# Multi-resolution-diffusion-recommender/SDRM

Hardware: AMD Instinct MI355X
Metric: denoising-steps/sec (train+sample) on ML-1M latents (higher is better)
Workload: dtype f32; 1 GPU; ML-1M/MLP shaped synthetic latents (C3/C4); latent=340, width=340, hidden_layers=1, global_batch=8192, n_sample=5429, step_mix=15 train : 78 sample per job cycle, rng=philox4x32-10 on device, sampler_row_chains=2, parallelism=user-sharded dp1, collectives=none

## Files before the change

### include/sdrm_hip_debug.h

```cpp
#ifndef SDRM_HIP_DEBUG_H
#define SDRM_HIP_DEBUG_H

#include "sdrm_hip.h"

#ifdef __cplusplus
extern "C" {
#endif

int sdrm_debug_device_check(const char* gcn_arch, int compute_units);

enum { SDRM_TILE_AUTO = -1, SDRM_TILE_COUNT = 5 };

int sdrm_debug_set_tile(sdrm_engine* e, int cfg);
int sdrm_debug_set_nt32_rows(sdrm_engine* e, int max_rows, int max_rows_train);
int sdrm_debug_set_skinny(sdrm_engine* e, int on);
int sdrm_debug_set_rowchain(sdrm_engine* e, int mode);
int sdrm_debug_set_rows48(sdrm_engine* e, int mode);
int sdrm_debug_set_rows48_split(sdrm_engine* e, int mode);
int sdrm_debug_rows48_split_available(const sdrm_engine* e);
int sdrm_debug_set_rows48_share(sdrm_engine* e, int on);
int sdrm_debug_set_sample_persist(sdrm_engine* e, int mode);
int sdrm_debug_split_skew(sdrm_engine* e, unsigned skew);
int sdrm_debug_set_wgrad_strips(sdrm_engine* e, int on);
int sdrm_debug_set_dgrad_rows(sdrm_engine* e, int mode);
int sdrm_debug_rowchain_available(const sdrm_engine* e);
int sdrm_debug_set_fused_reverse(sdrm_engine* e, int mode);
int sdrm_debug_set_chains(sdrm_engine* e, int chains);
int sdrm_debug_chains(const sdrm_engine* e);

int sdrm_debug_set_gradient_buckets(sdrm_engine* e, int buckets);

int sdrm_debug_philox_draws(sdrm_engine* e, uint64_t seed, uint32_t purpose, uint32_t step, int64_t row0, int rows, int quads,
                            float* normals, uint8_t* lowbits, void* stream);

void* sdrm_debug_comm_handle(const sdrm_engine* e);

int sdrm_debug_plan_wgrad(int rows, int n_out, int k_in, int* slices, int* rows_per_slice);

int sdrm_debug_gemm(int variant, int cfg, const float* A, const float* B, float* C, int M, int N, int K, void* stream);
int sdrm_debug_gemm_time(int variant, int cfg, int M, int N, int K, int reps, float* us_out, void* stream);

#ifdef __cplusplus
}
#endif
#endif
```

### sdrm_amd/_lib.py

```python
from __future__ import annotations

import ctypes as C
import os

from . import _build

_LIB = None

c_void_p, c_int, c_int64, c_uint64, c_float = C.c_void_p, C.c_int, C.c_int64, C.c_uint64, C.c_float


class TrainRandoms(C.Structure):
    _fields_ = [("noise", c_void_p), ("t", c_void_p), ("keep", c_void_p)]


class VaeDecoder(C.Structure):
    _fields_ = [("w1", c_void_p), ("b1", c_void_p), ("w2", c_void_p), ("b2", c_void_p), ("latent", c_int), ("hidden", c_int),
                ("n_items", c_int)]


class VaeEncoder(C.Structure):
    _fields_ = [("w1", c_void_p), ("b1", c_void_p), ("w2", c_void_p), ("b2", c_void_p), ("n_items", c_int), ("hidden", c_int),
                ("latent", c_int)]

# ... 74 lines not shown
    "sdrm_debug_set_skinny": (c_int, [c_void_p, c_int]),
    "sdrm_debug_set_rowchain": (c_int, [c_void_p, c_int]),
    "sdrm_debug_set_rows48": (c_int, [c_void_p, c_int]),
    "sdrm_debug_set_rows48_split": (c_int, [c_void_p, c_int]),
    "sdrm_debug_rows48_split_available": (c_int, [c_void_p]),
    "sdrm_debug_split_skew": (c_int, [c_void_p, C.c_uint32]),
    "sdrm_debug_set_sample_persist": (c_int, [c_void_p, c_int]),
    "sdrm_debug_set_rows48_share": (c_int, [c_void_p, c_int]),
    "sdrm_debug_rowchain_available": (c_int, [c_void_p]),
    "sdrm_debug_set_wgrad_strips": (c_int, [c_void_p, c_int]),
    "sdrm_debug_set_dgrad_rows": (c_int, [c_void_p, c_int]),
    "sdrm_debug_comm_handle": (c_void_p, [c_void_p]),
    "sdrm_debug_plan_wgrad": (c_int, [c_int, c_int, c_int, C.POINTER(c_int), C.POINTER(c_int)]),
    "sdrm_debug_gemm_time": (c_int, [c_int, c_int, c_int, c_int, c_int, c_int, C.POINTER(c_float), c_void_p]),
    "sdrm_debug_gemm": (c_int, [c_int, c_int, c_void_p, c_void_p, c_void_p, c_int, c_int, c_int, c_void_p]),
}

RNG_EXPLICIT, RNG_PHILOX = 0, 1
STATUS = {0: "SDRM_OK", -1: "SDRM_ERR_ARG", -2: "SDRM_ERR_SHAPE", -3: "SDRM_ERR_HIP", -4: "SDRM_ERR_STATE",
          -5: "SDRM_ERR_NOMEM", -6: "SDRM_ERR_RCCL", -7: "SDRM_ERR_DEVICE"}


def lib_path() -> str:
    return _build.LIB_PATH


def load(build_if_missing: bool = True):
    global _LIB
    if _LIB is not None:
        return _LIB
# ... 37 lines not shown
```

### sdrm_amd/csrc/gemm.h

```cpp
#pragma once
#include <hip/hip_runtime.h>
#include <stdint.h>

#include "bufres.h"

#include <type_traits>

#include "philox.h"
#include "select.h"

namespace sdrm {

typedef float f32x16 __attribute__((ext_vector_type(16)));

enum : int { LD_KCONTIG = 0, LD_MCONTIG = 1 };
enum : int { XF_NONE = 0, XF_PRELU = 1 };
enum : int {
  EPI_BIAS = 0,
  EPI_BIAS_TANH = 1,
  EPI_BIAS_TANH_G = 2,
  EPI_DPRELU = 3,
  EPI_SLAB = 4,
  EPI_PLAIN = 5,
  EPI_TANH_REV = 6,
// ... 23 lines not shown
  static constexpr int STAGE = STAGE_KMAJOR > STAGE_KMINOR ? STAGE_KMAJOR : STAGE_KMINOR;
  static_assert(WM_ * WN_ == 4, "4 waves per work-group");
  static_assert(MF_ == 32 || MF_ == 16, "MFMA tile edge");
  static_assert(TM >= 1 && TN >= 1, "wave tile must hold at least one MFMA tile");
};

template <int MF> struct AccT;
template <> struct AccT<32> { typedef float type __attribute__((ext_vector_type(16))); };
template <> struct AccT<16> { typedef float type __attribute__((ext_vector_type(4))); };

struct GemmArgs {
  const float* A; int lda; int limA;
  const float* B; int ldb; int limB;
  float* C; int ldc;
  int K;
  int kchunk;
  int tiles_n;
  int nblocks;
  int nsplits;
  uint32_t magic_tiles_n, magic_nblocks;
  const float* bias;
  const float* slopeA;
  const float* slopeB;
  const float* aux; int ldaux; const float* slopeE; float* slope_partial;
  size_t slab_stride; float* dbias; int dbias_stride;
  unsigned long long* stamps;
  int rows_valid, cols_valid;
  float* revX; float* revU; int rev_ldx, rev_s0, rev_n, rev_L, rev_step;
  float rev_c1, rev_sqrt_alpha, rev_sqrt_beta, rev_nd;
  uint32_t rev_seed_lo, rev_seed_hi, rev_call_id; int64_t rev_row0;
// ... 260 lines not shown
    if constexpr (PF_STATE) {
      const int rows_left = min(max(p.rev_n - p.rev_s0 - m0, 0), BM);
      const brsrc resX = make_brsrc(p.revX + (size_t)(p.rev_s0 + m0) * p.rev_ldx, (uint32_t)rows_left * (uint32_t)p.rev_ldx * 4u);
#pragma unroll
      for (int a = 0; a < TM; ++a)
#pragma unroll
        for (int b = 0; b < TN; ++b) {
          const int col = n0 + wn * (BN / Cfg::WN) + b * MF + l31;
          const int r0 = wm * (BM / Cfg::WM) + a * MF + 4 * lhi;
#pragma unroll
          for (int r = 0; r < NR; ++r)
            pf_x[a][b][r] = bload1a<COHA>(resX, (uint32_t)((r0 + ((MF == 32) ? (r & 3) + 8 * (r >> 2) : r)) * p.rev_ldx + col) * 4u, 0u);
        }
    }
  };
  const int aoffk = (wm * (BM / Cfg::WM) + l31) * LDK + ((MF == 32) ? (BK / 2) : 4) * lhi;
  const int boffk = (wn * (BN / Cfg::WN) + l31) * LDK + ((MF == 32) ? (BK / 2) : 4) * lhi;

  if constexpr (KM) {
    constexpr int NS = 4 * NQ;
    static_assert(NS >= 2 * NQ + 4, "not enough MFMA shadows for the pipeline pieces");
    float4 fa0[TM][NQ], fb0[TN][NQ], fa1[TM][NQ], fb1[TN][NQ];
    auto rd_all = [&](float4 (&fa)[TM][NQ], float4 (&fb)[TN][NQ], int stage) {
      const float* As = smem + stage * Cfg::STAGE;
      const float* Bs = As + BOFF;
#pragma unroll
      for (int q = 0; q < NQ; ++q) {
#pragma unroll
        for (int a = 0; a < TM; ++a) fa[a][q] = *reinterpret_cast<const float4*>(As + aoffk + MF * a * LDK + QSTEP * q);
#pragma unroll
        for (int b = 0; b < TN; ++b) fb[b][q] = *reinterpret_cast<const float4*>(Bs + boffk + MF * b * LDK + QSTEP * q);
      }
    };
    auto kstep = [&](auto active_tag, const float4 (&ca)[TM][NQ], const float4 (&cb)[TN][NQ], float4 (&na)[TM][NQ],
                     float4 (&nb)[TN][NQ], int rs, float4 (&xa)[NVA], float4 (&xb)[NVB], int ss, int li) {
      constexpr bool ACTIVE = decltype(active_tag)::value;
      const float* Ar = smem + rs * Cfg::STAGE;
      const float* Br = Ar + BOFF;
      float* Aw = smem + ss * Cfg::STAGE;
      const int k0 = kb + min(li, nt - 1) * BK;
#pragma unroll
      for (int sl = 0; sl < NS; ++sl) {
        const int q = sl >> 2, j = sl & 3;
        if constexpr (ACTIVE) {
#pragma unroll
          for (int a = 0; a < TM; ++a)
#pragma unroll
            for (int b = 0; b < TN; ++b) {
              const float av = j == 0 ? ca[a][q].x : j == 1 ? ca[a][q].y : j == 2 ? ca[a][q].z : ca[a][q].w;
              const float bv = j == 0 ? cb[b][q].x : j == 1 ? cb[b][q].y : j == 2 ? cb[b][q].z : cb[b][q].w;
              if constexpr (MF == 32) acc[a][b] = __builtin_amdgcn_mfma_f32_32x32x2f32(av, bv, acc[a][b], 0, 0, 0);
              else acc[a][b] = __builtin_amdgcn_mfma_f32_16x16x4f32(av, bv, acc[a][b], 0, 0, 0);
            }
        }
        if (sl < 2 * NQ) {
          if constexpr (ACTIVE) {
            const int rq = sl >> 1;
            if ((sl & 1) == 0) {
#pragma unroll
              for (int a = 0; a < TM; ++a) na[a][rq] = *reinterpret_cast<const float4*>(Ar + aoffk + MF * a * LDK + QSTEP * rq);
            } else {
#pragma unroll
              for (int b = 0; b < TN; ++b) nb[b][rq] = *reinterpret_cast<const float4*>(Br + boffk + MF * b * LDK + QSTEP * rq);
            }
          }
        } else if (sl == 2 * NQ) {
          if constexpr (XFA == XF_PRELU) prelu_regs<NVA>(xa, slopeA);
          else DIAG_ST((store_tile_km<XF_NONE, BM, LDK, BK>(Aw, xa, 0.f, tid)));
        } else if (sl == 2 * NQ + 1) {
          if constexpr (XFA == XF_PRELU) DIAG_ST((store_tile_km<XF_NONE, BM, LDK, BK>(Aw, xa, 0.f, tid)));
          DIAG_ST((store_tile_km<XFB, BN, LDK, BK>(Aw + BOFF, xb, slopeB, tid)));
        } else if (sl == 2 * NQ + 2) {
          DIAG_LD((load_tile<LOADA, BM, BK, COHA>(resA, voA, p.lda, k0 - kb, xa)));
        } else if (sl == 2 * NQ + 3) {
          DIAG_LD((load_tile<LOADB, BN, BK>(resB, voB, p.ldb, k0 - kb, xb)));
        }
        __builtin_amdgcn_sched_barrier(0);
      }
      DIAG_BAR();
    };
    if (nt > 0) {
      if constexpr (Cfg::PF == 2) {
        ld(ra0, rb0, 0);
        ld(ra1, rb1, 1);
#if defined(SDRM_STAMPS) && SDRM_STAMPS == 2
        t_ld = __builtin_amdgcn_s_memtime();
        __builtin_amdgcn_sched_barrier(0);
#endif
        epi_prefetch();
        if constexpr (EPI == EPI_TANH_REV) rev_draw();
        st(ra0, rb0, 0);
#if defined(SDRM_STAMPS) && SDRM_STAMPS == 2
        __builtin_amdgcn_sched_barrier(0);
        t_land = __builtin_amdgcn_s_memtime();
#endif
        ld(ra0, rb0, 2);
        st(ra1, rb1, 1);
        ld(ra1, rb1, 3);
      } else {
        ld(ra0, rb0, 0);
        epi_prefetch();
        if constexpr (EPI == EPI_TANH_REV) rev_draw();
        st(ra0, rb0, 0);
        ld(ra0, rb0, 1);
        st(ra0, rb0, 1);
        ld(ra0, rb0, 2);
      }
      __syncthreads();
#ifdef SDRM_STAMPS
      if (true) t_pro = __builtin_amdgcn_s_memtime();
#endif
      if (wave_active) rd_all(fa0, fb0, 0);
      __syncthreads();
      auto run = [&](auto tag) {
        int i = 0;
        for (; i + 1 < nt; i += 2) {
          if constexpr (Cfg::PF == 2) {
            kstep(tag, fa0, fb0, fa1, fb1, 1, ra0, rb0, 0, i + 4);
            kstep(tag, fa1, fb1, fa0, fb0, 0, ra1, rb1, 1, i + 5);
          } else {
            kstep(tag, fa0, fb0, fa1, fb1, 1, ra0, rb0, 0, i + 3);
            kstep(tag, fa1, fb1, fa0, fb0, 0, ra0, rb0, 1, i + 4);
          }
        }
        if (i < nt) kstep(tag, fa0, fb0, fa1, fb1, 1, ra0, rb0, 0, i + 4);
      };
      if (wave_active) run(std::true_type{});
      else run(std::false_type{});
    }
  } else {
    constexpr int G = BK / KG;
    static_assert(G >= 8, "pipeline pieces need 8 MFMA shadows");
    float ka0[TM][G], kb0[TN][G], ka1[TM][G], kb1[TN][G];
    auto col_sum = [&](int stage) {
      const float* As = smem + stage * Cfg::STAGE;
#pragma unroll
      for (int k = 0; k < BK; ++k) dbsum += As[k * LDA + tid];
    };
    auto kstep = [&](auto active_tag, const float (&ca)[TM][G], const float (&cb)[TN][G], float (&na)[TM][G],
                     float (&nb)[TN][G], int rs, float4 (&xa)[NVA], float4 (&xb)[NVB], int ss, int li, bool next_valid) {
// ... 224 lines not shown
```

### sdrm_amd/csrc/sdrm_hip.hip

```cpp
#include <hip/hip_runtime.h>

#include <algorithm>
#include <cmath>
#include <cstdio>
#include <cstdlib>
#include <cstring>
#include <mutex>
#include <set>
#include <string>
#include <type_traits>
#include <utility>
#include <vector>

#include "../../include/sdrm_hip.h"
#include "../../include/sdrm_hip_debug.h"
#include "compact.h"
#include "decode.h"
#include "elementwise.h"
#include "encode.h"
#include "exchange.h"
#include "feed.h"
#include "gemm.h"
#include "rank.h"
#include "rowchain.h"
// ... 332 lines not shown
    default: return launch_gemm_cfg<Cfg0, LA, LB, XA, XB, EPI>(a, M, N, splits, st, pr);
  }
}

template <int XA, int EPI>
hipError_t gemm_forward(GemmArgs a, const float* A, int lda, const float* Wc, int ldw, int M, int N, int K,
                        hipStream_t st, Prof pr, int cfg) {
  a.A = A; a.lda = lda; a.limA = M;
  a.B = Wc; a.ldb = ldw; a.limB = N;
  a.K = K; a.kchunk = K;
  return launch_gemm<LD_KCONTIG, LD_KCONTIG, XA, XF_NONE, EPI>(a, M, N, 1, st, pr, cfg);
}

hipError_t gemm_dgrad(sdrm_engine* e, const float* dC, int lddc, const float* WT, int ldwt, int M, int Nout, int Kin,
                      float* out, const float* aux, const float* slopeE, float* partial, hipStream_t st, double flops,
                      int cfg) {
  GemmArgs a{};
  a.A = dC; a.lda = lddc; a.limA = M;
  a.B = WT; a.ldb = ldwt; a.limB = Kin;
  a.C = out; a.ldc = e->WP;
  a.K = Nout; a.kchunk = Nout;
  a.aux = aux; a.ldaux = e->WP; a.slopeE = slopeE; a.slope_partial = partial;
  return launch_gemm<LD_KCONTIG, LD_KCONTIG, XF_NONE, XF_NONE, EPI_DPRELU>(a, M, Kin, 1, st, Prof{e, PC_DGRAD, flops}, cfg);
}

template <int XB>
hipError_t gemm_wgrad(const float* dC, int lddc, int Nout, const float* Act, int ldact, int Kin, const float* slopeB,
                      int Mrows, int S, int kchunk, float* slab, float* dbias, hipStream_t st, Prof pr, int cfg) {
  GemmArgs a{};
  a.A = dC; a.lda = lddc; a.limA = Nout;
  a.B = Act; a.ldb = ldact; a.limB = Kin;
  a.C = slab; a.ldc = Kin;
  a.K = Mrows; a.kchunk = kchunk;
  a.slopeB = slopeB;
  a.slab_stride = (size_t)Nout * Kin;
  a.dbias = dbias; a.dbias_stride = Nout;
// ... 512 lines not shown
struct NetView { const float *W0c, *Whc, *Woc, *bhc, *boc, *B0tab, *slope0, *slopeh; };
NetView snapshot_view(const sdrm_engine* e) {
  const float* b = e->smp_w;
  return NetView{b + e->smp_off[0], b + e->smp_off[1], b + e->smp_off[2], b + e->smp_off[3], b + e->smp_off[4], b + e->smp_off[5],
                 b + e->smp_off[6], b + e->smp_off[6] + 1};
}

int hidden_forward(sdrm_engine* e, int MP, int rows, hipStream_t st, int cfg, int r0 = 0, int cls = PC_FWD_HIDDEN,
                   bool post_act = false, const NetView* nv = nullptr) {
  const double fl = 2.0 * rows * (double)e->W * e->W;
  const size_t ro = (size_t)r0 * e->WP;
  for (int k = 1; k <= e->H; ++k) {
    if (post_act) {
      GemmArgs a{};
      a.C = (nv ? smp_buf(e, k) : pre_buf(e, k)) + ro; a.ldc = e->WP; a.bias = nv ? nv->bhc : e->bhc; a.slopeE = nv ? nv->slopeh : slope_ptr(e, k);
      HIP_TRY(e, (gemm_forward<XF_NONE, EPI_BIAS_PRELU>(a, (nv ? smp_buf(e, k - 1) : pre_buf(e, k - 1)) + ro, e->WP, nv ? nv->Whc : e->Whc, e->WP, MP, e->WP, e->WP,
                                                         st, Prof{e, cls, fl}, cfg)));
      continue;
    }
    GemmArgs a{};
    a.C = pre_buf(e, k) + ro; a.ldc = e->WP; a.bias = e->bhc; a.slopeA = slope_ptr(e, k - 1);
    HIP_TRY(e, (gemm_forward<XF_PRELU, EPI_BIAS>(a, pre_buf(e, k - 1) + ro, e->WP, e->Whc, e->WP, MP, e->WP, e->WP, st,
                                                 Prof{e, cls, fl}, cfg)));
  }
  return SDRM_OK;
}

int upload_schedule(sdrm_engine* e, float beta1, float beta2) {
  const int T = e->T, n = T + 1;
  std::vector<float> b(n), al(n), ab(n), sq(n), om(n);
  const float step = 1.0f / (float)T;
  float run = 0.f;
  for (int i = 0; i < n; ++i) {
    const float lin = (i < n / 2) ? (0.f + step * (float)i) : (1.f - step * (float)(n - 1 - i));
    b[i] = (beta2 - beta1) * lin + beta1;
    al[i] = 1.f - b[i];
// ... 484 lines not shown
    pa.mode = mode; pa.seed_lo = (uint32_t)seed; pa.seed_hi = (uint32_t)(seed >> 32); pa.step = (uint32_t)step;
    pa.row0 = row0; pa.nd = nd;
    {
      pa.emb = emb_args(e);
      e->tables_fresh = true;
      pa.emb_row0 = B + (MP - 3 * B);
      pa.emb_chunks = (e->WP + 63) / 64;
      pa.emb_blocks = (e->T + 1) * pa.emb_chunks;
      const int main_blocks = (int)(((int64_t)pa.emb_row0 * (e->K0 / 4) + 255) / 256);
      SDRM_LAUNCH(e, k_prep_train, dim3(pa.emb_blocks + main_blocks), dim3(256), 2 * e->T * sizeof(float), st, pa);
      HIP_TRY(e, hipGetLastError());
    }
    {
      GemmArgs a{};
      a.C = pre_buf(e, 0); a.ldc = e->WP; a.bias = e->B0tab; a.ldtab = e->WP; a.trow = e->tdev; a.trow_B = B;
      HIP_TRY(e, (gemm_forward<XF_NONE, EPI_BIAS_ROWTAB>(a, e->U, e->K0, e->W0c, e->K0, MP, e->WP, e->LP, st,
                                                         Prof{e, PC_FWD_L0, 2.0 * 3 * B * (double)e->W * e->L}, cfg)));
    }
    int rc = hidden_forward(e, MP, 3 * B, st, cfg);
    if (rc) return rc;
    {
      GemmArgs a{};
      a.C = e->Y; a.ldc = e->LP; a.bias = e->boc; a.slopeA = slope_ptr(e, e->H);
      a.rows_valid = MP; a.cols_valid = e->LP;
      HIP_TRY(e, (gemm_forward<XF_PRELU, EPI_BIAS_TANH>(a, pre_buf(e, e->H), e->WP, e->Woc, e->WP, MP, e->LP, e->WP, st,
                                                        Prof{e, PC_FWD_OUT, 2.0 * 3 * B * (double)e->L * e->W}, cfg)));
    }
    LossArgs la{};
    la.Y = e->Y; la.x0 = x0; la.B = B; la.L = e->L; la.LP = e->LP; la.part = e->loss_part;
    SDRM_LAUNCH(e, k_loss_partials, dim3(LOSS_BLOCKS), dim3(1024), 0, st, la);
    HIP_TRY(e, hipGetLastError());
  }
  if (!fold_sums) {
    SDRM_LAUNCH(e, k_loss_sums, dim3(1), dim3(256), 0, st, (const double*)e->loss_part, p.loss_parts, (double)B * (double)e->L,
                       sums ? sums : e->sums);
    HIP_TRY(e, hipGetLastError());
  }
  e->fwd_x0 = x0; e->fwd_done = true;
  return SDRM_OK;
// ... 56 lines not shown
    }
    case StepPlan::ROWS_PER_LAYER: {
      dgrad_blocks = p.groups;
      int rc = launch_dgrad_rows(e, e->dY, e->WofT, pre_buf(e, H), slope_ptr(e, H), dpre_buf(e, H),
                                 e->alpha_part + (size_t)H * e->alpha_part_stride, p.groups, flO, st);
      for (int k = H; k >= 1 && !rc; --k)
        rc = launch_dgrad_rows(e, dpre_buf(e, k), e->WhfT, pre_buf(e, k - 1), slope_ptr(e, k - 1), dpre_buf(e, k - 1),
                               e->alpha_part + (size_t)(k - 1) * e->alpha_part_stride, p.groups, flH, st);
      if (rc) return rc;
      break;
    }
    case StepPlan::TILES: {
      const int cfg_d = choose_cfg(e->tune, MP, e->tune.nt32_max_rows_train);
      dgrad_blocks = ((MP + kCfgBM[cfg_d] - 1) / kCfgBM[cfg_d]) * ((e->WP + kCfgBN[cfg_d] - 1) / kCfgBN[cfg_d]);
      HIP_TRY(e, gemm_dgrad(e, e->dY, e->LP, e->WocT, e->LP, MP, e->LP, e->WP, dpre_buf(e, H), pre_buf(e, H), slope_ptr(e, H),
                            e->alpha_part + (size_t)H * e->alpha_part_stride, st, flO, cfg_d));
      for (int k = H; k >= 1; --k)
        HIP_TRY(e, gemm_dgrad(e, dpre_buf(e, k), e->WP, e->WhcT, e->WP, MP, e->WP, e->WP, dpre_buf(e, k - 1), pre_buf(e, k - 1),
                              slope_ptr(e, k - 1), e->alpha_part + (size_t)(k - 1) * e->alpha_part_stride, st, flH, cfg_d));
      break;
    }
  }
  if (with_wgrad0)
    HIP_TRY(e, (gemm_wgrad<XF_NONE>(dpre_buf(e, 0), e->WP, e->WP, e->U, e->K0, e->K0, nullptr, MP, S0, kc0, e->slab0, e->db0s, st,
                                    Prof{e, PC_WGRAD_L0, fl0}, cfg_w)));
  e->bwd_S0 = e->bwd_SH = e->bwd_SO = S0; e->bwd_kc0 = e->bwd_kcH = e->bwd_kcO = kc0;
  e->bwd_dgrad_blocks = dgrad_blocks;
  return SDRM_OK;
}

int backward_wgrads(sdrm_engine* e, hipStream_t st, bool with_wgrad0) {
  const StepPlan& p = e->plan;
  if (p.path == StepPlan::SKINNY) return SDRM_OK;
  const int B = p.B, MP = p.MP, H = e->H, SH = e->bwd_SH, SO = e->bwd_SO;
// ... 518 lines not shown
  c.path = skinny_net(e) ? SampleCall::SKINNY
           : sample_persist_fits(e, n, c.MP, multires, mode, c.chains) ? SampleCall::PERSIST : SampleCall::PER_LAYER;
  c.i_next = i_first;
  c.persist_phase = 0;
  c.active = true;
  rc = c.path == SampleCall::SKINNY ? launch_skinny_sampler(e, c, st) : launch_sample_init(e, c, st);
  if (rc) c.active = false;
  return rc;
}

namespace {
int launch_sample_persist(sdrm_engine* e, SampleCall& s, int count, hipStream_t st) {
  const NetView nv = snapshot_view(e);
  const int MP = s.MP, tiles_m = MP / 32, tiles_n = e->WP / 32;
  SamplePersistArgs P{};
  auto layer = [&](GemmArgs& a, const float* A, int lda, const float* Wc, int ldw, float* C, int ldc, int K) {
    a.A = A; a.lda = lda; a.limA = MP; a.B = Wc; a.ldb = ldw; a.limB = e->WP; a.K = K; a.kchunk = K; a.C = C; a.ldc = ldc;
    return gemm_set_grid(a, tiles_m, tiles_n, 1);
  };
  bool ok = layer(P.l0, e->Us, e->LP, nv.W0c, e->K0, smp_buf(e, 0), e->WP, e->LP);
  P.l0.slopeE = nv.slope0;
  ok = ok && layer(P.lh, smp_buf(e, 0), e->WP, nv.Whc, e->WP, smp_buf(e, 1), e->WP, e->WP);
  P.lh.bias = nv.bhc; P.lh.slopeE = nv.slopeh;
  ok = ok && layer(P.lo, smp_buf(e, e->H), e->WP, nv.Woc, e->WP, e->smp_Y, e->LP, e->WP);
  if (!ok) return fail(e, SDRM_ERR_SHAPE, "persistent sampler: grid beyond the tile arithmetic");
  GemmArgs& a = P.lo;
  a.bias = nv.boc; a.rows_valid = MP; a.cols_valid = e->LP;
  a.revX = e->X; a.revU = e->Us; a.rev_ldx = e->LP; a.rev_s0 = 0; a.rev_n = s.n; a.rev_L = e->L; a.rev_nd = s.nd;
  a.rev_seed_lo = (uint32_t)s.seed; a.rev_seed_hi = (uint32_t)(s.seed >> 32); a.rev_call_id = (uint32_t)s.call_id; a.rev_row0 = s.row0;
  P.pre_stride = (size_t)e->MPmax * e->WP;
  P.B0tab = nv.B0tab; P.ldtab = e->WP; P.rev = e->rev_dev;
  P.T = e->T; P.H = e->H; P.i_first = s.i_next; P.count = count;
  P.row_tiles = tiles_m; P.tiles_n = tiles_n;
  P.cnt = e->xcntS; P.base = s.persist_phase * (uint32_t)tiles_n; P.abort_ = e->xabort_dev;
  const int steps = std::min(count, s.i_next);
  s.persist_phase += (uint32_t)(steps * (e->H + 2));
  const int grid = 8 * tiles_n * ((tiles_m + 7) / 8);
  const double flops = 2.0 * s.n * ((double)e->W * e->L + (double)e->H * e->W * e->W + (double)e->L * e->W) * steps;
  const int rc = hip_rc(e, "k_sample_persist", profiled(e, PC_SMP_PERSIST, flops, st, [&] {
    SDRM_LAUNCH(e, (k_sample_persist<Cfg4>), dim3((unsigned)grid), dim3(NTHREADS), 0, st, P);
    return hipGetLastError();
  }));
  if (rc) return rc;
  s.i_next -= steps;
  return SDRM_OK;
}

int sample_chain_step(sdrm_engine* e, const SampleCall& s, const NetView& nv, int i, int s0, int s1, hipStream_t sc) {
  const int L = e->L, rows = s1 - s0, MP = round_up(rows, BM);
  const size_t nL = (size_t)s.n * L;
  const int cfg = choose_cfg(e->tune, MP, e->tune.nt32_max_rows);
  GemmArgs a0{};
  a0.C = smp_buf(e, 0) + (size_t)s0 * e->WP; a0.ldc = e->WP; a0.bias = nv.B0tab + (size_t)i * e->WP; a0.slopeE = nv.slope0;
  HIP_TRY(e, (gemm_forward<XF_NONE, EPI_BIAS_PRELU>(a0, e->Us + (size_t)s0 * e->LP, e->LP, nv.W0c, e->K0, MP, e->WP, e->LP, sc,
                                                    Prof{e, PC_SMP_L0, 2.0 * rows * (double)e->W * e->L}, cfg)));
  int rc = hidden_forward(e, MP, rows, sc, cfg, s0, PC_SMP_HIDDEN, true, &nv);
  if (rc) return rc;
  float c1, sqrt_alpha, sqrt_beta;
  reverse_coeffs(e, i, c1, sqrt_alpha, sqrt_beta);
  const bool fused = s.mode == SDRM_RNG_PHILOX && (e->tune.fuse_rev == 2 || (e->tune.fuse_rev == 1 && rows <= FUSE_REV_MAX_ROWS));
  GemmArgs a{};
  a.C = e->smp_Y + (size_t)s0 * e->LP; a.ldc = e->LP; a.bias = nv.boc;
  a.rows_valid = MP; a.cols_valid = e->LP;
  const Prof pr{e, PC_SMP_OUT, 2.0 * rows * (double)e->L * e->W};
  if (fused) {
    a.revX = e->X; a.revU = e->Us; a.rev_ldx = e->LP; a.rev_s0 = s0; a.rev_n = s1; a.rev_L = L; a.rev_step = i;
    a.rev_c1 = c1; a.rev_sqrt_alpha = sqrt_alpha; a.rev_sqrt_beta = sqrt_beta; a.rev_nd = s.nd;
    a.rev_seed_lo = (uint32_t)s.seed; a.rev_seed_hi = (uint32_t)(s.seed >> 32); a.rev_call_id = (uint32_t)s.call_id;
    a.rev_row0 = s.row0; a.rev_rowid = s.multires ? e->rowid_dev : nullptr;
    HIP_TRY(e, (gemm_forward<XF_NONE, EPI_TANH_REV>(a, smp_buf(e, e->H) + (size_t)s0 * e->WP, e->WP, nv.Woc, e->WP, MP, e->LP, e->WP, sc, pr, cfg)));
    return SDRM_OK;
  }
  HIP_TRY(e, (gemm_forward<XF_NONE, EPI_BIAS_TANH>(a, smp_buf(e, e->H) + (size_t)s0 * e->WP, e->WP, nv.Woc, e->WP, MP, e->LP, e->WP, sc, pr, cfg)));
  ReverseArgs ra{};
  ra.X = e->X; ra.Y = e->smp_Y; ra.U = e->Us;
  ra.Z = (s.mode == SDRM_RNG_EXPLICIT && i > 1) ? s.z + (size_t)i * nL : nullptr;
  ra.keep_next = (s.mode == SDRM_RNG_EXPLICIT && i > 1) ? s.keep + (size_t)(i - 1) * nL : nullptr;
  ra.Tj = s.multires ? e->Tj_dev : nullptr;
// ... 513 lines not shown
    const int c = e->prof_cls[i];
    e->prof_ms[c] += ms; e->prof_fl[c] += e->prof_flops[i]; e->prof_n[c] += 1;
  }
  return SDRM_OK;
}

int sdrm_profile_get(const sdrm_engine* e, int cls, double* total_ms, int64_t* launches, double* flops) {
  if (!e || cls < 0 || cls >= PC_COUNT) return SDRM_ERR_ARG;
  if (total_ms) *total_ms = e->prof_ms[cls];
  if (launches) *launches = e->prof_n[cls];
  if (flops) *flops = e->prof_fl[cls];
  return SDRM_OK;
}

int sdrm_debug_gemm(int variant, int cfg, const float* A, const float* B, float* C, int M, int N, int K, void* stream) {
  if (!A || !B || !C || cfg < 0 || cfg >= N_TILE_CFGS) return SDRM_ERR_ARG;
  if (M % 32 || N % 32 || K % 32 || variant < 0 || variant > 2) return SDRM_ERR_SHAPE;
  hipStream_t st = (hipStream_t)stream;
  const int Mp = round_up(M, 128), Np = round_up(N, 128), Kp = round_up(K, 128);
  const int ar = variant == 2 ? Kp : Mp, ac = variant == 2 ? Mp : K;
  const int br = variant == 0 ? Np : Kp, bc = variant == 0 ? K : Np;
  float *dA = nullptr, *dB = nullptr, *dC = nullptr;
  if (dalloc(&dA, (size_t)ar * ac) != hipSuccess || dalloc(&dB, (size_t)br * bc) != hipSuccess ||
      dalloc(&dC, (size_t)Mp * Np) != hipSuccess)
    return SDRM_ERR_NOMEM;
  const int a_rows = variant == 2 ? K : M, a_cols = variant == 2 ? M : K;
  const int b_rows = variant == 0 ? N : K, b_cols = variant == 0 ? K : N;
  hipError_t rc = hipMemcpy2DAsync(dA, (size_t)ac * 4, A, (size_t)a_cols * 4, (size_t)a_cols * 4, a_rows, hipMemcpyDeviceToDevice, st);
  if (rc == hipSuccess)
    rc = hipMemcpy2DAsync(dB, (size_t)bc * 4, B, (size_t)b_cols * 4, (size_t)b_cols * 4, b_rows, hipMemcpyDeviceToDevice, st);
  GemmArgs a{};
  a.C = dC; a.ldc = Np; a.K = K; a.kchunk = K;
  a.A = dA; a.lda = ac; a.limA = M; a.B = dB; a.ldb = bc; a.limB = N;
  if (rc == hipSuccess) {
    const Prof np{nullptr, 0, 0.0};
    if (variant == 0) rc = launch_gemm<LD_KCONTIG, LD_KCONTIG, XF_NONE, XF_NONE, EPI_PLAIN>(a, M, N, 1, st, np, cfg);
    else if (variant == 1) rc = launch_gemm<LD_KCONTIG, LD_MCONTIG, XF_NONE, XF_NONE, EPI_PLAIN>(a, M, N, 1, st, np, cfg);
    else rc = launch_gemm<LD_MCONTIG, LD_MCONTIG, XF_NONE, XF_NONE, EPI_PLAIN>(a, M, N, 1, st, np, cfg);
  }
  if (rc == hipSuccess)
    rc = hipMemcpy2DAsync(C, (size_t)N * 4, dC, (size_t)Np * 4, (size_t)N * 4, M, hipMemcpyDeviceToDevice, st);
  if (rc == hipSuccess) rc = hipStreamSynchronize(st);
  (void)hipFree(dA); (void)hipFree(dB); (void)hipFree(dC);
  return rc == hipSuccess ? SDRM_OK : SDRM_ERR_HIP;
}

#ifdef SDRM_STAMPS
// ... 78 lines not shown
```

### sdrm_amd/csrc/wgrad2.h

```cpp
#pragma once
#include <hip/hip_runtime.h>
#include <stdint.h>

#include "bufres.h"
#include "gemm.h"

#ifndef WG2_DIAG
#define WG2_DIAG 0
#endif

namespace sdrm {

constexpr int WG2_MAX_PROBLEMS = 8;
constexpr int WG2_MAX_UNITS = 32;
constexpr int WG2_BK = 16;

struct Wg2Problem {
  const float* A; int lda;
  const float* B; int ldb;
  float* slab; int ldc;
  size_t slab_stride;
};

struct Wg2Strip { int8_t problem; int8_t ktile; };
// ... 2 lines not shown
  Wg2Problem p[WG2_MAX_PROBLEMS];
  Wg2Strip strip[WG2_MAX_UNITS][4];
  int units, slices, rows, kchunk;
};

__device__ __forceinline__ Wg2Problem wg2_problem(const Wg2Args& a, int idx) {
  Wg2Problem r = a.p[0];
#pragma unroll
  for (int p = 1; p < WG2_MAX_PROBLEMS; ++p)
    if (p == idx) r = a.p[p];
  return r;
}

template <int NT>
struct Wg2Cfg {
  static constexpr int WP = 32 * NT, LDA = WP + 4, LDB = 32 + 4;
  static constexpr int A_TILE = WG2_BK * LDA, B_TILE = WG2_BK * LDB;
  static constexpr int STAGE = 2 * A_TILE + 4 * B_TILE;
  static constexpr size_t LDS_BYTES = 2 * (size_t)STAGE * 4;
  static constexpr int NA4 = WG2_BK * WP / 4, NB4 = 4 * WG2_BK * 32 / 4;
  static constexpr int NLA = (NA4 + NTHREADS - 1) / NTHREADS, NLB = NB4 / NTHREADS;
  static_assert(NLB == 2, "two B blocks per half work-group");
  static_assert(LDS_BYTES <= 160 * 1024, "stages do not fit LDS");
};

template <int NT>
__global__ __launch_bounds__(NTHREADS, 1) void k_wgrad_strips(const Wg2Args a) {
  typedef Wg2Cfg<NT> C;
  constexpr int WP = C::WP, LDA = C::LDA, LDB = C::LDB, BK = WG2_BK;
  __shared__ __attribute__((aligned(16))) float smem[2 * C::STAGE];
  const int tid = threadIdx.x, lane = tid & 63;
  const int wave = __builtin_amdgcn_readfirstlane(tid >> 6);
  const int l31 = lane & 31, lhi = lane >> 5;
  const int logical = xcd_remap((int)blockIdx.x, a.units * a.slices);
  const int slice = logical / a.units, unit = logical - slice * a.units;
  const int m_begin = slice * a.kchunk, m_end = min(m_begin + a.kchunk, a.rows);
  const int nt = (m_end - m_begin) / BK;

  const Wg2Strip st = a.strip[unit][wave];
  const int pa = a.strip[unit][0].problem;
  int pb = pa;
#pragma unroll
  for (int w = 1; w < 4; ++w)
    if (a.strip[unit][w].problem >= 0) pb = a.strip[unit][w].problem;
  const bool two = pb != pa;
// ... 67 lines not shown
  auto lstore = [&](auto two_tag, const RSet& r, int stage) __attribute__((always_inline)) {
    constexpr int NPC = (decltype(two_tag)::value ? 2 * C::NLA : C::NLA) + C::NLB;
#pragma unroll
    for (int k = 0; k < NPC; ++k) lstore_piece(two_tag, r, smem + stage * C::STAGE, k);
  };

  f32x16 acc[NT];
#pragma unroll
  for (int t = 0; t < NT; ++t)
#pragma unroll
    for (int r = 0; r < 16; ++r) acc[t][r] = 0.f;

  const int aoff = ai * C::A_TILE + lhi * LDA + l31;
  const int boff = 2 * C::A_TILE + wave * C::B_TILE + lhi * LDB + l31;

  auto kstep = [&](auto two_tag, int i, RSet& nx) __attribute__((always_inline)) {
    constexpr int NPC = (decltype(two_tag)::value ? 2 * C::NLA : C::NLA) + C::NLB;
    constexpr int NSLOT = (BK / 2) * NT, HALF = NSLOT / 2;
    constexpr int STRIDE = HALF / NPC >= 1 ? HALF / NPC : 1;
    static_assert(NPC <= HALF, "more staging pieces than MFMA slots");
    const float* S = smem + (i & 1) * C::STAGE;
    float* Sn = smem + ((i + 1) & 1) * C::STAGE;
    const int m4 = m_begin + min(i + 4, nt - 1) * BK;
    float fa0[NT], fa1[NT], fb0 = 0.f, fb1 = 0.f;
#pragma unroll
    for (int t = 0; t < NT; ++t) fa0[t] = S[aoff + 32 * t];
    fb0 = S[boff];
#pragma unroll
    for (int g = 0; g < BK / 2; ++g) {
      float (&ca)[NT] = (g & 1) ? fa1 : fa0;
      float (&na)[NT] = (g & 1) ? fa0 : fa1;
      const float cb = (g & 1) ? fb1 : fb0;
      float& nb = (g & 1) ? fb0 : fb1;
#pragma unroll
      for (int t = 0; t < NT; ++t) {
        if (!(WG2_DIAG & 1)) acc[t] = __builtin_amdgcn_mfma_f32_32x32x2f32(ca[t], cb, acc[t], 0, 0, 0);
        if (g + 1 < BK / 2 && !(WG2_DIAG & 8)) {
          if (t == 0) nb = S[boff + 2 * (g + 1) * LDB];
          na[t] = S[aoff + 2 * (g + 1) * LDA + 32 * t];
        }
        const int slot = g * NT + t;
        if (slot < HALF) {
          if (slot % STRIDE == 0 && slot / STRIDE < NPC && !(WG2_DIAG & 2)) lstore_piece(two_tag, nx, Sn, slot / STRIDE);
        } else {
          const int s2 = slot - HALF;
          if (s2 % STRIDE == 0 && s2 / STRIDE < NPC && !(WG2_DIAG & 4)) gload_piece(two_tag, nx, m4, s2 / STRIDE);
        }
        __builtin_amdgcn_sched_barrier(0);
      }
    }
    __syncthreads();
  };
  auto run = [&](auto two_tag) __attribute__((always_inline)) {
    gload(two_tag, r0, 0);
    lstore(two_tag, r0, 0);
    gload(two_tag, r1, 1); gload(two_tag, r2, 2); gload(two_tag, r0, 3);
    __syncthreads();
    int i = 0;
    for (; i + 2 < nt; i += 3) {
      kstep(two_tag, i, r1);
      kstep(two_tag, i + 1, r2);
      kstep(two_tag, i + 2, r0);
    }
    if (i < nt) kstep(two_tag, i, r1);
    if (i + 1 < nt) kstep(two_tag, i + 1, r2);
  };
  if (nt > 0) {
    if (two) run(std::true_type{});
    else run(std::false_type{});
  }

  if (!active) return;
  const Wg2Problem P = wg2_problem(a, st.problem);
  float* __restrict__ dst = P.slab + (size_t)slice * P.slab_stride + (size_t)(4 * lhi) * P.ldc + 32 * st.ktile + l31;
#pragma unroll
  for (int t = 0; t < NT; ++t)
#pragma unroll
    for (int r = 0; r < 16; ++r) dst[(size_t)(32 * t + (r & 3) + 8 * (r >> 2)) * P.ldc] = acc[t][r];
}

// ... 18 lines not shown
```

Before: 9118 denoising-steps/s.

## Skip padded K tail in GEMM last tiles and triple-buffer wgrad strips

Adds a k_valid field so the MF=16 forward and dgrad GEMMs can peel the last two K tiles and skip MFMAs and LDS reads over the zero-padded tail when only a few real K columns remain (340 padded up). Separately, the wgrad strip kernel moves from two to three LDS stages. Each kstep now prefetches the first fragments of the next stage, loads run one tile further ahead, and B padding is removed. This aims to cut wasted MFMA work on padding and to hide LDS latency, at the cost of more LDS use and more code specialisation. It also adds a debug entry point for testing k_valid.

```diff
diff --git a/include/sdrm_hip_debug.h b/include/sdrm_hip_debug.h
--- a/include/sdrm_hip_debug.h
+++ b/include/sdrm_hip_debug.h
@@ -38,6 +38,7 @@
 int sdrm_debug_plan_wgrad(int rows, int n_out, int k_in, int* slices, int* rows_per_slice);
 
 int sdrm_debug_gemm(int variant, int cfg, const float* A, const float* B, float* C, int M, int N, int K, void* stream);
+int sdrm_debug_gemm_kvalid(int variant, int cfg, const float* A, const float* B, float* C, int M, int N, int K, int k_valid, void* stream);
 int sdrm_debug_gemm_time(int variant, int cfg, int M, int N, int K, int reps, float* us_out, void* stream);
 
 #ifdef __cplusplus
diff --git a/sdrm_amd/_lib.py b/sdrm_amd/_lib.py
--- a/sdrm_amd/_lib.py
+++ b/sdrm_amd/_lib.py
@@ -112,6 +112,7 @@
     "sdrm_debug_plan_wgrad": (c_int, [c_int, c_int, c_int, C.POINTER(c_int), C.POINTER(c_int)]),
     "sdrm_debug_gemm_time": (c_int, [c_int, c_int, c_int, c_int, c_int, c_int, C.POINTER(c_float), c_void_p]),
     "sdrm_debug_gemm": (c_int, [c_int, c_int, c_void_p, c_void_p, c_void_p, c_int, c_int, c_int, c_void_p]),
+    "sdrm_debug_gemm_kvalid": (c_int, [c_int, c_int, c_void_p, c_void_p, c_void_p, c_int, c_int, c_int, c_int, c_void_p]),
 }
 
 RNG_EXPLICIT, RNG_PHILOX = 0, 1
diff --git a/sdrm_amd/csrc/gemm.h b/sdrm_amd/csrc/gemm.h
--- a/sdrm_amd/csrc/gemm.h
+++ b/sdrm_amd/csrc/gemm.h
@@ -61,6 +61,7 @@
   const float* B; int ldb; int limB;
   float* C; int ldc;
   int K;
+  int k_valid;
   int kchunk;
   int tiles_n;
   int nblocks;
@@ -351,6 +352,18 @@
         }
     }
   };
+  constexpr bool CAN_COMPACT = (MF == 16) && (EPI != EPI_SLAB) && (LOADA == LD_KCONTIG && LOADB == LD_KCONTIG);
+  const int k_top = p.k_valid - (ke - 16);
+  const bool compact = CAN_COMPACT && nt >= 2 && (ke - kb) == nt * BK && k_top >= 1 && k_top <= 4;
+  const int aoffc = (wm * (BM / Cfg::WM) + l31) * LDK + (BK - 16) + lhi;
+  const int boffc = (wn * (BN / Cfg::WN) + l31) * LDK + (BK - 16) + lhi;
+  auto epi_front = [&]() {
+    if constexpr (EPI == EPI_TANH_REV) {
+      rev_draw();
+      __builtin_amdgcn_sched_barrier(0);
+    }
+    epi_prefetch();
+  };
   const int aoffk = (wm * (BM / Cfg::WM) + l31) * LDK + ((MF == 32) ? (BK / 2) : 4) * lhi;
   const int boffk = (wn * (BN / Cfg::WN) + l31) * LDK + ((MF == 32) ? (BK / 2) : 4) * lhi;
 
@@ -369,9 +382,10 @@
         for (int b = 0; b < TN; ++b) fb[b][q] = *reinterpret_cast<const float4*>(Bs + boffk + MF * b * LDK + QSTEP * q);
       }
     };
-    auto kstep = [&](auto active_tag, const float4 (&ca)[TM][NQ], const float4 (&cb)[TN][NQ], float4 (&na)[TM][NQ],
+    auto kstep = [&](auto active_tag, auto next_tag, auto this_tag, const float4 (&ca)[TM][NQ], const float4 (&cb)[TN][NQ], float4 (&na)[TM][NQ],
                      float4 (&nb)[TN][NQ], int rs, float4 (&xa)[NVA], float4 (&xb)[NVB], int ss, int li) {
       constexpr bool ACTIVE = decltype(active_tag)::value;
+      constexpr bool NEXT_COMPACT = decltype(next_tag)::value, THIS_COMPACT = decltype(this_tag)::value;
       const float* Ar = smem + rs * Cfg::STAGE;
       const float* Br = Ar + BOFF;
       float* Aw = smem + ss * Cfg::STAGE;
@@ -379,7 +393,7 @@
 #pragma unroll
       for (int sl = 0; sl < NS; ++sl) {
         const int q = sl >> 2, j = sl & 3;
-        if constexpr (ACTIVE) {
+        if (ACTIVE && !(THIS_COMPACT && q == NQ - 1 && j > 0)) {
 #pragma unroll
           for (int a = 0; a < TM; ++a)
 #pragma unroll
@@ -393,12 +407,19 @@
         if (sl < 2 * NQ) {
           if constexpr (ACTIVE) {
             const int rq = sl >> 1;
+            const bool one = NEXT_COMPACT && rq == NQ - 1;
             if ((sl & 1) == 0) {
 #pragma unroll
-              for (int a = 0; a < TM; ++a) na[a][rq] = *reinterpret_cast<const float4*>(Ar + aoffk + MF * a * LDK + QSTEP * rq);
+              for (int a = 0; a < TM; ++a) {
+                if (one) na[a][rq].x = Ar[aoffc + MF * a * LDK];
+                else na[a][rq] = *reinterpret_cast<const float4*>(Ar + aoffk + MF * a * LDK + QSTEP * rq);
+              }
             } else {
 #pragma unroll
-              for (int b = 0; b < TN; ++b) nb[b][rq] = *reinterpret_cast<const float4*>(Br + boffk + MF * b * LDK + QSTEP * rq);
+              for (int b = 0; b < TN; ++b) {
+                if (one) nb[b][rq].x = Br[boffc + MF * b * LDK];
+                else nb[b][rq] = *reinterpret_cast<const float4*>(Br + boffk + MF * b * LDK + QSTEP * rq);
+              }
             }
           }
         } else if (sl == 2 * NQ) {
@@ -424,8 +445,7 @@
         t_ld = __builtin_amdgcn_s_memtime();
         __builtin_amdgcn_sched_barrier(0);
 #endif
-        epi_prefetch();
-        if constexpr (EPI == EPI_TANH_REV) rev_draw();
+        epi_front();
         st(ra0, rb0, 0);
 #if defined(SDRM_STAMPS) && SDRM_STAMPS == 2
         __builtin_amdgcn_sched_barrier(0);
@@ -436,8 +456,7 @@
         ld(ra1, rb1, 3);
       } else {
         ld(ra0, rb0, 0);
-        epi_prefetch();
-        if constexpr (EPI == EPI_TANH_REV) rev_draw();
+        epi_front();
         st(ra0, rb0, 0);
         ld(ra0, rb0, 1);
         st(ra0, rb0, 1);
@@ -449,18 +468,36 @@
 #endif
       if (wave_active) rd_all(fa0, fb0, 0);
       __syncthreads();
+      constexpr int AHEAD = Cfg::PF == 2 ? 4 : 3;
+      auto even = [&](auto tag, auto next_tag, auto this_tag, int i) { kstep(tag, next_tag, this_tag, fa0, fb0, fa1, fb1, 1, ra0, rb0, 0, i + AHEAD); };
+      auto odd = [&](auto tag, auto next_tag, auto this_tag, int i) {
+        if constexpr (Cfg::PF == 2) kstep(tag, next_tag, this_tag, fa1, fb1, fa0, fb0, 0, ra1, rb1, 1, i + AHEAD);
+        else kstep(tag, next_tag, this_tag, fa1, fb1, fa0, fb0, 0, ra0, rb0, 1, i + AHEAD);
+      };
       auto run = [&](auto tag) {
+        constexpr bool PEEL = decltype(tag)::value && CAN_COMPACT;
+        const std::false_type no{};
+        const std::true_type yes{};
+        const int n_main = (PEEL && compact) ? nt - 2 : nt;
         int i = 0;
-        for (; i + 1 < nt; i += 2) {
-          if constexpr (Cfg::PF == 2) {
-            kstep(tag, fa0, fb0, fa1, fb1, 1, ra0, rb0, 0, i + 4);
-            kstep(tag, fa1, fb1, fa0, fb0, 0, ra1, rb1, 1, i + 5);
-          } else {
-            kstep(tag, fa0, fb0, fa1, fb1, 1, ra0, rb0, 0, i + 3);
-            kstep(tag, fa1, fb1, fa0, fb0, 0, ra0, rb0, 1, i + 4);
+        for (; i + 1 < n_main; i += 2) {
+          even(tag, no, no, i);
+          odd(tag, no, no, i + 1);
+        }
+        if constexpr (PEEL) {
+          if (compact) {
+            if (i < n_main) {
+              even(tag, no, no, i);
+              odd(tag, yes, no, i + 1);
+              even(tag, no, yes, i + 2);
+            } else {
+              even(tag, yes, no, i);
+              odd(tag, no, yes, i + 1);
+            }
+            return;
           }
         }
-        if (i < nt) kstep(tag, fa0, fb0, fa1, fb1, 1, ra0, rb0, 0, i + 4);
+        if (i < nt) even(tag, no, no, i);
       };
       if (wave_active) run(std::true_type{});
       else run(std::false_type{});
diff --git a/sdrm_amd/csrc/sdrm_hip.hip b/sdrm_amd/csrc/sdrm_hip.hip
--- a/sdrm_amd/csrc/sdrm_hip.hip
+++ b/sdrm_amd/csrc/sdrm_hip.hip
@@ -370,12 +370,12 @@
 
 hipError_t gemm_dgrad(sdrm_engine* e, const float* dC, int lddc, const float* WT, int ldwt, int M, int Nout, int Kin,
                       float* out, const float* aux, const float* slopeE, float* partial, hipStream_t st, double flops,
-                      int cfg) {
+                      int cfg, int nout_valid) {
   GemmArgs a{};
   a.A = dC; a.lda = lddc; a.limA = M;
   a.B = WT; a.ldb = ldwt; a.limB = Kin;
   a.C = out; a.ldc = e->WP;
-  a.K = Nout; a.kchunk = Nout;
+  a.K = Nout; a.kchunk = Nout; a.k_valid = nout_valid;
   a.aux = aux; a.ldaux = e->WP; a.slopeE = slopeE; a.slope_partial = partial;
   return launch_gemm<LD_KCONTIG, LD_KCONTIG, XF_NONE, XF_NONE, EPI_DPRELU>(a, M, Kin, 1, st, Prof{e, PC_DGRAD, flops}, cfg);
 }
@@ -918,12 +918,14 @@
     if (post_act) {
       GemmArgs a{};
       a.C = (nv ? smp_buf(e, k) : pre_buf(e, k)) + ro; a.ldc = e->WP; a.bias = nv ? nv->bhc : e->bhc; a.slopeE = nv ? nv->slopeh : slope_ptr(e, k);
+      a.k_valid = e->W;
       HIP_TRY(e, (gemm_forward<XF_NONE, EPI_BIAS_PRELU>(a, (nv ? smp_buf(e, k - 1) : pre_buf(e, k - 1)) + ro, e->WP, nv ? nv->Whc : e->Whc, e->WP, MP, e->WP, e->WP,
                                                          st, Prof{e, cls, fl}, cfg)));
       continue;
     }
     GemmArgs a{};
     a.C = pre_buf(e, k) + ro; a.ldc = e->WP; a.bias = e->bhc; a.slopeA = slope_ptr(e, k - 1);
+    a.k_valid = e->W;
     HIP_TRY(e, (gemm_forward<XF_PRELU, EPI_BIAS>(a, pre_buf(e, k - 1) + ro, e->WP, e->Whc, e->WP, MP, e->WP, e->WP, st,
                                                  Prof{e, cls, fl}, cfg)));
   }
@@ -1438,6 +1440,7 @@
     {
       GemmArgs a{};
       a.C = pre_buf(e, 0); a.ldc = e->WP; a.bias = e->B0tab; a.ldtab = e->WP; a.trow = e->tdev; a.trow_B = B;
+      a.k_valid = e->L;
       HIP_TRY(e, (gemm_forward<XF_NONE, EPI_BIAS_ROWTAB>(a, e->U, e->K0, e->W0c, e->K0, MP, e->WP, e->LP, st,
                                                          Prof{e, PC_FWD_L0, 2.0 * 3 * B * (double)e->W * e->L}, cfg)));
     }
@@ -1446,7 +1449,7 @@
     {
       GemmArgs a{};
       a.C = e->Y; a.ldc = e->LP; a.bias = e->boc; a.slopeA = slope_ptr(e, e->H);
-      a.rows_valid = MP; a.cols_valid = e->LP;
+      a.rows_valid = MP; a.cols_valid = e->LP; a.k_valid = e->W;
       HIP_TRY(e, (gemm_forward<XF_PRELU, EPI_BIAS_TANH>(a, pre_buf(e, e->H), e->WP, e->Woc, e->WP, MP, e->LP, e->WP, st,
                                                         Prof{e, PC_FWD_OUT, 2.0 * 3 * B * (double)e->L * e->W}, cfg)));
     }
@@ -1533,10 +1536,10 @@
       const int cfg_d = choose_cfg(e->tune, MP, e->tune.nt32_max_rows_train);
       dgrad_blocks = ((MP + kCfgBM[cfg_d] - 1) / kCfgBM[cfg_d]) * ((e->WP + kCfgBN[cfg_d] - 1) / kCfgBN[cfg_d]);
       HIP_TRY(e, gemm_dgrad(e, e->dY, e->LP, e->WocT, e->LP, MP, e->LP, e->WP, dpre_buf(e, H), pre_buf(e, H), slope_ptr(e, H),
-                            e->alpha_part + (size_t)H * e->alpha_part_stride, st, flO, cfg_d));
+                            e->alpha_part + (size_t)H * e->alpha_part_stride, st, flO, cfg_d, e->L));
       for (int k = H; k >= 1; --k)
         HIP_TRY(e, gemm_dgrad(e, dpre_buf(e, k), e->WP, e->WhcT, e->WP, MP, e->WP, e->WP, dpre_buf(e, k - 1), pre_buf(e, k - 1),
-                              slope_ptr(e, k - 1), e->alpha_part + (size_t)(k - 1) * e->alpha_part_stride, st, flH, cfg_d));
+                              slope_ptr(e, k - 1), e->alpha_part + (size_t)(k - 1) * e->alpha_part_stride, st, flH, cfg_d, e->W));
       break;
     }
   }
@@ -2085,15 +2088,15 @@
   const NetView nv = snapshot_view(e);
   const int MP = s.MP, tiles_m = MP / 32, tiles_n = e->WP / 32;
   SamplePersistArgs P{};
-  auto layer = [&](GemmArgs& a, const float* A, int lda, const float* Wc, int ldw, float* C, int ldc, int K) {
-    a.A = A; a.lda = lda; a.limA = MP; a.B = Wc; a.ldb = ldw; a.limB = e->WP; a.K = K; a.kchunk = K; a.C = C; a.ldc = ldc;
+  auto layer = [&](GemmArgs& a, const float* A, int lda, const float* Wc, int ldw, float* C, int ldc, int K, int k_valid) {
+    a.A = A; a.lda = lda; a.limA = MP; a.B = Wc; a.ldb = ldw; a.limB = e->WP; a.K = K; a.kchunk = K; a.k_valid = k_valid; a.C = C; a.ldc = ldc;
     return gemm_set_grid(a, tiles_m, tiles_n, 1);
   };
-  bool ok = layer(P.l0, e->Us, e->LP, nv.W0c, e->K0, smp_buf(e, 0), e->WP, e->LP);
+  bool ok = layer(P.l0, e->Us, e->LP, nv.W0c, e->K0, smp_buf(e, 0), e->WP, e->LP, e->L);
   P.l0.slopeE = nv.slope0;
-  ok = ok && layer(P.lh, smp_buf(e, 0), e->WP, nv.Whc, e->WP, smp_buf(e, 1), e->WP, e->WP);
+  ok = ok && layer(P.lh, smp_buf(e, 0), e->WP, nv.Whc, e->WP, smp_buf(e, 1), e->WP, e->WP, e->W);
   P.lh.bias = nv.bhc; P.lh.slopeE = nv.slopeh;
-  ok = ok && layer(P.lo, smp_buf(e, e->H), e->WP, nv.Woc, e->WP, e->smp_Y, e->LP, e->WP);
+  ok = ok && layer(P.lo, smp_buf(e, e->H), e->WP, nv.Woc, e->WP, e->smp_Y, e->LP, e->WP, e->W);
   if (!ok) return fail(e, SDRM_ERR_SHAPE, "persistent sampler: grid beyond the tile arithmetic");
   GemmArgs& a = P.lo;
   a.bias = nv.boc; a.rows_valid = MP; a.cols_valid = e->LP;
@@ -2123,6 +2126,7 @@
   const int cfg = choose_cfg(e->tune, MP, e->tune.nt32_max_rows);
   GemmArgs a0{};
   a0.C = smp_buf(e, 0) + (size_t)s0 * e->WP; a0.ldc = e->WP; a0.bias = nv.B0tab + (size_t)i * e->WP; a0.slopeE = nv.slope0;
+  a0.k_valid = e->L;
   HIP_TRY(e, (gemm_forward<XF_NONE, EPI_BIAS_PRELU>(a0, e->Us + (size_t)s0 * e->LP, e->LP, nv.W0c, e->K0, MP, e->WP, e->LP, sc,
                                                     Prof{e, PC_SMP_L0, 2.0 * rows * (double)e->W * e->L}, cfg)));
   int rc = hidden_forward(e, MP, rows, sc, cfg, s0, PC_SMP_HIDDEN, true, &nv);
@@ -2132,7 +2136,7 @@
   const bool fused = s.mode == SDRM_RNG_PHILOX && (e->tune.fuse_rev == 2 || (e->tune.fuse_rev == 1 && rows <= FUSE_REV_MAX_ROWS));
   GemmArgs a{};
   a.C = e->smp_Y + (size_t)s0 * e->LP; a.ldc = e->LP; a.bias = nv.boc;
-  a.rows_valid = MP; a.cols_valid = e->LP;
+  a.rows_valid = MP; a.cols_valid = e->LP; a.k_valid = e->W;
   const Prof pr{e, PC_SMP_OUT, 2.0 * rows * (double)e->L * e->W};
   if (fused) {
     a.revX = e->X; a.revU = e->Us; a.rev_ldx = e->LP; a.rev_s0 = s0; a.rev_n = s1; a.rev_L = L; a.rev_step = i;
@@ -2676,8 +2680,12 @@
 }
 
 int sdrm_debug_gemm(int variant, int cfg, const float* A, const float* B, float* C, int M, int N, int K, void* stream) {
+  return sdrm_debug_gemm_kvalid(variant, cfg, A, B, C, M, N, K, K, stream);
+}
+
+int sdrm_debug_gemm_kvalid(int variant, int cfg, const float* A, const float* B, float* C, int M, int N, int K, int k_valid, void* stream) {
   if (!A || !B || !C || cfg < 0 || cfg >= N_TILE_CFGS) return SDRM_ERR_ARG;
-  if (M % 32 || N % 32 || K % 32 || variant < 0 || variant > 2) return SDRM_ERR_SHAPE;
+  if (M % 32 || N % 32 || K % 32 || variant < 0 || variant > 2 || k_valid < 1 || k_valid > K) return SDRM_ERR_SHAPE;
   hipStream_t st = (hipStream_t)stream;
   const int Mp = round_up(M, 128), Np = round_up(N, 128), Kp = round_up(K, 128);
   const int ar = variant == 2 ? Kp : Mp, ac = variant == 2 ? Mp : K;
@@ -2692,7 +2700,7 @@
   if (rc == hipSuccess)
     rc = hipMemcpy2DAsync(dB, (size_t)bc * 4, B, (size_t)b_cols * 4, (size_t)b_cols * 4, b_rows, hipMemcpyDeviceToDevice, st);
   GemmArgs a{};
-  a.C = dC; a.ldc = Np; a.K = K; a.kchunk = K;
+  a.C = dC; a.ldc = Np; a.K = K; a.kchunk = K; a.k_valid = k_valid;
   a.A = dA; a.lda = ac; a.limA = M; a.B = dB; a.ldb = bc; a.limB = N;
   if (rc == hipSuccess) {
     const Prof np{nullptr, 0, 0.0};
diff --git a/sdrm_amd/csrc/wgrad2.h b/sdrm_amd/csrc/wgrad2.h
--- a/sdrm_amd/csrc/wgrad2.h
+++ b/sdrm_amd/csrc/wgrad2.h
@@ -40,21 +40,26 @@
 
 template <int NT>
 struct Wg2Cfg {
-  static constexpr int WP = 32 * NT, LDA = WP + 4, LDB = 32 + 4;
+  static constexpr int WP = 32 * NT, LDA = WP + 4, LDB = 32;
   static constexpr int A_TILE = WG2_BK * LDA, B_TILE = WG2_BK * LDB;
   static constexpr int STAGE = 2 * A_TILE + 4 * B_TILE;
-  static constexpr size_t LDS_BYTES = 2 * (size_t)STAGE * 4;
+  static constexpr int NSTAGE = 3;
+  static constexpr size_t LDS_BYTES = NSTAGE * (size_t)STAGE * 4;
   static constexpr int NA4 = WG2_BK * WP / 4, NB4 = 4 * WG2_BK * 32 / 4;
   static constexpr int NLA = (NA4 + NTHREADS - 1) / NTHREADS, NLB = NB4 / NTHREADS;
   static_assert(NLB == 2, "two B blocks per half work-group");
+  static_assert(LDA % 4 == 0 && LDB % 4 == 0 && A_TILE % 4 == 0 && B_TILE % 4 == 0, "ds_write_b128 alignment");
   static_assert(LDS_BYTES <= 160 * 1024, "stages do not fit LDS");
 };
+static_assert(Wg2Cfg<4>::LDS_BYTES <= 160 * 1024 && Wg2Cfg<5>::LDS_BYTES <= 160 * 1024 && Wg2Cfg<6>::LDS_BYTES <= 160 * 1024 &&
+              Wg2Cfg<7>::LDS_BYTES <= 160 * 1024 && Wg2Cfg<8>::LDS_BYTES <= 160 * 1024 && Wg2Cfg<9>::LDS_BYTES <= 160 * 1024 &&
+              Wg2Cfg<10>::LDS_BYTES <= 160 * 1024 && Wg2Cfg<11>::LDS_BYTES <= 160 * 1024, "three stages must fit LDS for every strip width");
 
 template <int NT>
 __global__ __launch_bounds__(NTHREADS, 1) void k_wgrad_strips(const Wg2Args a) {
   typedef Wg2Cfg<NT> C;
   constexpr int WP = C::WP, LDA = C::LDA, LDB = C::LDB, BK = WG2_BK;
-  __shared__ __attribute__((aligned(16))) float smem[2 * C::STAGE];
+  __shared__ __attribute__((aligned(16))) float smem[C::NSTAGE * C::STAGE];
   const int tid = threadIdx.x, lane = tid & 63;
   const int wave = __builtin_amdgcn_readfirstlane(tid >> 6);
   const int l31 = lane & 31, lhi = lane >> 5;
@@ -152,56 +157,68 @@
   const int aoff = ai * C::A_TILE + lhi * LDA + l31;
   const int boff = 2 * C::A_TILE + wave * C::B_TILE + lhi * LDB + l31;
 
-  auto kstep = [&](auto two_tag, int i, RSet& nx) __attribute__((always_inline)) {
+  float fa0[NT], fb0 = 0.f;
+  auto kstep = [&](auto two_tag, auto stage_tag, int i, RSet& nx) __attribute__((always_inline)) {
     constexpr int NPC = (decltype(two_tag)::value ? 2 * C::NLA : C::NLA) + C::NLB;
     constexpr int NSLOT = (BK / 2) * NT, HALF = NSLOT / 2;
     constexpr int STRIDE = HALF / NPC >= 1 ? HALF / NPC : 1;
+    constexpr int STG = decltype(stage_tag)::value;
     static_assert(NPC <= HALF, "more staging pieces than MFMA slots");
-    const float* S = smem + (i & 1) * C::STAGE;
-    float* Sn = smem + ((i + 1) & 1) * C::STAGE;
-    const int m4 = m_begin + min(i + 4, nt - 1) * BK;
-    float fa0[NT], fa1[NT], fb0 = 0.f, fb1 = 0.f;
-#pragma unroll
-    for (int t = 0; t < NT; ++t) fa0[t] = S[aoff + 32 * t];
-    fb0 = S[boff];
+    const float* S = smem + STG * C::STAGE;
+    const float* Sf = smem + ((STG + 1) % C::NSTAGE) * C::STAGE;
+    float* Sn = smem + ((STG + 2) % C::NSTAGE) * C::STAGE;
+    const int m5 = m_begin + min(i + 5, nt - 1) * BK;
+    float fa1[NT], fb1 = 0.f;
 #pragma unroll
     for (int g = 0; g < BK / 2; ++g) {
       float (&ca)[NT] = (g & 1) ? fa1 : fa0;
       float (&na)[NT] = (g & 1) ? fa0 : fa1;
       const float cb = (g & 1) ? fb1 : fb0;
       float& nb = (g & 1) ? fb0 : fb1;
+      const float* R = (g + 1 < BK / 2) ? S + 2 * (g + 1) * LDA : Sf;
+      const float* Rb = (g + 1 < BK / 2) ? S + 2 * (g + 1) * LDB : Sf;
 #pragma unroll
       for (int t = 0; t < NT; ++t) {
         if (!(WG2_DIAG & 1)) acc[t] = __builtin_amdgcn_mfma_f32_32x32x2f32(ca[t], cb, acc[t], 0, 0, 0);
-        if (g + 1 < BK / 2 && !(WG2_DIAG & 8)) {
-          if (t == 0) nb = S[boff + 2 * (g + 1) * LDB];
-          na[t] = S[aoff + 2 * (g + 1) * LDA + 32 * t];
+        if (g == 0 && t == 0) __builtin_amdgcn_sched_barrier(0);
+        if (!(WG2_DIAG & 8)) {
+          if (t == 0) nb = Rb[boff];
+          na[t] = R[aoff + 32 * t];
         }
         const int slot = g * NT + t;
         if (slot < HALF) {
           if (slot % STRIDE == 0 && slot / STRIDE < NPC && !(WG2_DIAG & 2)) lstore_piece(two_tag, nx, Sn, slot / STRIDE);
         } else {
           const int s2 = slot - HALF;
-          if (s2 % STRIDE == 0 && s2 / STRIDE < NPC && !(WG2_DIAG & 4)) gload_piece(two_tag, nx, m4, s2 / STRIDE);
+          if (s2 % STRIDE == 0 && s2 / STRIDE < NPC && !(WG2_DIAG & 4)) gload_piece(two_tag, nx, m5, s2 / STRIDE);
         }
         __builtin_amdgcn_sched_barrier(0);
       }
     }
     __syncthreads();
+    __builtin_amdgcn_sched_barrier(0);
   };
   auto run = [&](auto two_tag) __attribute__((always_inline)) {
+    typedef std::integral_constant<int, 0> S0;
+    typedef std::integral_constant<int, 1> S1;
+    typedef std::integral_constant<int, 2> S2;
     gload(two_tag, r0, 0);
+    gload(two_tag, r1, 1);
     lstore(two_tag, r0, 0);
-    gload(two_tag, r1, 1); gload(two_tag, r2, 2); gload(two_tag, r0, 3);
+    lstore(two_tag, r1, 1);
+    gload(two_tag, r2, 2); gload(two_tag, r0, 3); gload(two_tag, r1, 4);
     __syncthreads();
+#pragma unroll
+    for (int t = 0; t < NT; ++t) fa0[t] = smem[aoff + 32 * t];
+    fb0 = smem[boff];
     int i = 0;
     for (; i + 2 < nt; i += 3) {
-      kstep(two_tag, i, r1);
-      kstep(two_tag, i + 1, r2);
-      kstep(two_tag, i + 2, r0);
+      kstep(two_tag, S0{}, i, r2);
+      kstep(two_tag, S1{}, i + 1, r0);
+      kstep(two_tag, S2{}, i + 2, r1);
     }
-    if (i < nt) kstep(two_tag, i, r1);
-    if (i + 1 < nt) kstep(two_tag, i + 1, r2);
+    if (i < nt) kstep(two_tag, S0{}, i, r2);
+    if (i + 1 < nt) kstep(two_tag, S1{}, i + 1, r0);
   };
   if (nt > 0) {
     if (two) run(std::true_type{});
```

After: 9200 denoising-steps/s (median of 6 runs). About the same (+0.9%).
